# GuoleiSun/VSS-CFFM

Measured on AMD Instinct MI355X. Metric: clips/sec (fwd+bwd) CFFM-B1 480x480 T=4 hot path (CFFA+CFM, decoder_focal depth 2), higher is better.
Workload: dtype f32 in/out, f32 accumulate; MFMA operands: split-bf16 (hi+lo, ~2^-17) in the Linear GEMMs, f16 in QK^T/AV

## Files before the change

### vss_cffm_amd/csrc/cffa_kernels.h

```cpp
#pragma once
#include "cffm_common.h"

__device__ __forceinline__ void transpose_body(const float* __restrict__ src, float* __restrict__ dst,
                                               int rows, int cols, long src_bs, long dst_bs,
                                               const float* __restrict__ addend, int add_mod, int add_skip,
                                               float* __restrict__ copy_dst, int bx, int by, int bz) {
    __shared__ float tile[64][65];
    const int r0 = by * 64, c0 = bx * 64;
    const float* s = src + (long)bz * src_bs;
    float* d = dst + (long)bz * dst_bs;
    const int q = threadIdx.x & 15, p = threadIdx.x >> 4;
    const bool vin = (cols % 4 == 0) && (src_bs % 4 == 0) && (((uintptr_t)src & 15) == 0);
    const bool vout = (rows % 4 == 0) && (dst_bs % 4 == 0) && (((uintptr_t)dst & 15) == 0) && (((uintptr_t)addend & 15) == 0);
    const float* ad = (addend && (bz % add_mod) != add_skip) ? addend + (long)bz * dst_bs : nullptr;
    float* cp = (copy_dst && (bz % add_mod) != add_skip) ? copy_dst + (long)bz * src_bs : nullptr;
#pragma unroll
    for (int k = 0; k < 4; ++k) {
        const int r = r0 + p + 16 * k, c = c0 + 4 * q;
        f32x4 v = (f32x4){0.f, 0.f, 0.f, 0.f};
        if (r < rows) {
            if (vin && c + 3 < cols) {
                v = *(const f32x4*)(s + (long)r * cols + c);
                if (cp) *(f32x4*)(cp + (long)r * cols + c) = v;
            } else
// ... 265 lines not shown
    }
    f32x4 ag = (f32x4){0.f, 0.f, 0.f, 0.f}, ab = (f32x4){0.f, 0.f, 0.f, 0.f};
    __syncthreads();
#pragma unroll
    for (int k = 0; k < LNB_PIX; ++k) {
        const int i = s + LNB_SPLIT * (wave + LNB_WAVES * k);
        if (i >= CFFM_WA) break;
        const int y = 7 * wy + i / 7, x = 7 * wx + i % 7;
        if (!((y < G.H0) && (x < G.W0))) continue;
        const long pix = (long)y * G.W0 + x;
        const float rs = rsr[k];
        const f32x4 xh = (xr[k] - mur[k]) * rs;
        const f32x4 z = xh * gm + bt;
        const f32x4 dz = dzr[k] + m0[k] * dp;
        const float dm = wave_sum_hi(dot4(dp, z));
        if (lane == 63) sdM[i] = dm;
        ag += dz * xh;
        ab += dz;
        const f32x4 gz = dz * gm;
        const float m1 = wave_sum(gz[0] + gz[1] + gz[2] + gz[3]) * (1.f / CFFM_C);
        const float m2 = wave_sum(dot4(gz, xh)) * (1.f / CFFM_C);
        const f32x4 dx = (gz - m1 - xh * m2) * rs + addr[k];
        *(f32x4*)(dxf + pix * CFFM_C + 4 * lane) = dx;
    }
    *(f32x4*)(&red[wave][0][4 * lane]) = ag;
    *(f32x4*)(&red[wave][1][4 * lane]) = ab;
    __syncthreads();
    float* r = rec + (long)blockIdx.x * LNP_RSTRIDE;
    for (int e = threadIdx.x; e < 2 * CFFM_C; e += LNB_THREADS) {
        const int which = e / CFFM_C, ch = e % CFFM_C;
        float t = red[0][which][ch];
#pragma unroll
        for (int q = 1; q < LNB_WAVES; ++q) t += red[q][which][ch];
        r[e] = t;
    }
    if (threadIdx.x < CFFM_WA) r[2 * CFFM_C + threadIdx.x] = sdM[threadIdx.x];
    if (threadIdx.x == CFFM_WA) r[2 * CFFM_C + CFFM_WA] = sbs;
}

#define RB_MAXD 4
struct CffaRefBlocks {
    int n;
    const float* gamma[RB_MAXD];
    const float* beta[RB_MAXD];
    const float* M[RB_MAXD];
    const float* dzall[RB_MAXD];
    float* rec[RB_MAXD];
};
#define RB_LDS_BLOCK (14 * CFFM_C + 2 * 14 * CFFM_WA)
__host__ __device__ constexpr int cffa_ref_lds(int D) {
    return 4 * ((D * RB_LDS_BLOCK > LNB_WAVES * D * 2 * CFFM_C + 14 * D * CFFM_WA ? D * RB_LDS_BLOCK : LNB_WAVES * D * 2 * CFFM_C + 14 * D * CFFM_WA) + 4 * D + 4);
}

struct RefRows { f32x4 x[LNB_PIX], add[LNB_PIX]; float mu[LNB_PIX], rs[LNB_PIX]; };
template <bool ACC>
__device__ __forceinline__ void ln_pool_ref_load(RefRows& R, const Geo& G, const float* __restrict__ xf, const float* __restrict__ dxf,
                                                 const float* __restrict__ mean_f, const float* __restrict__ rstd_f, int s, int wy, int wx,
                                                 int lane, int wave) {
#pragma unroll
    for (int k = 0; k < LNB_PIX; ++k) {
        const int i = s + LNB_SPLIT * (wave + LNB_WAVES * k);
        const int y = 7 * wy + i / 7, x = 7 * wx + i % 7;
        R.x[k] = R.add[k] = (f32x4){0.f, 0.f, 0.f, 0.f};
        R.mu[k] = R.rs[k] = 0.f;
        if (i < CFFM_WA && y < G.H0 && x < G.W0) {
            const long pix = (long)y * G.W0 + x;
            R.x[k] = *(const f32x4*)(xf + pix * CFFM_C + 4 * lane);
            R.mu[k] = mean_f[pix];
            R.rs[k] = rstd_f[pix];
            if (ACC) R.add[k] = *(const f32x4*)(dxf + pix * CFFM_C + 4 * lane);
        }
    }
}
template <int NC, int D>
__device__ __forceinline__ void ln_pool_bwd_ref_frame(const Geo& G, const RefRows& R, float* __restrict__ dxf,
                                                      const float* sP, const float* sMm, float* sdM, const f32x4 (&gm)[D], const f32x4 (&bt)[D],
                                                      f32x4 (&ag)[D], f32x4 (&ab)[D], int g0, int s, int wy, int wx, int lane, int wave) {
#pragma unroll
    for (int k = 0; k < LNB_PIX; ++k) {
        const int i = s + LNB_SPLIT * (wave + LNB_WAVES * k);
        if (i >= CFFM_WA) break;
        const int y = 7 * wy + i / 7, x = 7 * wx + i % 7;
        if (!((y < G.H0) && (x < G.W0))) continue;
        const long pix = (long)y * G.W0 + x;
        const float rs = R.rs[k];
        const f32x4 xh = (R.x[k] - R.mu[k]) * rs;
        f32x4 gz = (f32x4){0.f, 0.f, 0.f, 0.f};
        constexpr int NCD = NC == 9 ? 3 : (NC == 4 ? 2 : 1), WSG = NC == 9 ? 2 : (NC == 4 ? 3 : 7);
        const int iy = i / 7, ix = i % 7;
        int u0 = 0, u1 = 0, v0 = 0, v1 = 0;
        if (NC > 1) {
            u0 = (iy > 0 ? iy - 1 : 0) / WSG; u1 = (iy < 5 ? iy : 5) / WSG;
            v0 = (ix > 0 ? ix - 1 : 0) / WSG; v1 = (ix < 5 ? ix : 5) / WSG;
        }
#pragma unroll
        for (int d = 0; d < D; ++d) {
            const f32x4 z = xh * gm[d] + bt[d];
            f32x4 dz = (f32x4){0.f, 0.f, 0.f, 0.f};
            for (int u = u0; u <= u1; ++u)
                for (int v = v0; v <= v1; ++v) {
                    const int c = d * 14 + g0 - 1 + u * NCD + v;
                    const f32x4 dp = *(const f32x4*)(sP + c * CFFM_C + 4 * lane);
                    dz += sMm[c * CFFM_WA + i] * dp;
                    const float dm = wave_sum_hi(dot4(dp, z));
                    if (lane == 63) sdM[c * CFFM_WA + i] = dm;
                }
            ag[d] += dz * xh;
            ab[d] += dz;
            gz += dz * gm[d];
        }
        const float m1 = wave_sum(gz[0] + gz[1] + gz[2] + gz[3]) * (1.f / CFFM_C);
        const float m2 = wave_sum(dot4(gz, xh)) * (1.f / CFFM_C);
        const f32x4 dx = (gz - m1 - xh * m2) * rs + R.add[k];
        *(f32x4*)(dxf + pix * CFFM_C + 4 * lane) = dx;
    }
}

template <int D, bool ACC>
__global__ void __launch_bounds__(LNB_THREADS) k_ln_pool_bwd_ref(Geo G, const float* __restrict__ x_ref, long ref_bs, CffaRefBlocks Bk,
                                                                 const float* __restrict__ mean_in, const float* __restrict__ rstd_in,
                                                                 float* __restrict__ dx_ref, long dref_bs) {
    CFFM_DYN_SMEM(smem);
    float* sP = (float*)smem;
    float* sMm = sP + D * 14 * CFFM_C;
    float* red = (float*)smem;
    constexpr int body = D * (14 * CFFM_C + 14 * CFFM_WA), redn = LNB_WAVES * D * 2 * CFFM_C;
    float* sdM = (float*)smem + (body > redn ? body : redn);
    float* sbs = sdM + D * 14 * CFFM_WA;
    const int s = blockIdx.x % LNB_SPLIT, wb = blockIdx.x / LNB_SPLIT;
    const int w = wb % G.nW, b = wb / G.nW;
    const int wy = w / G.gx, wx = w % G.gx;
    const int lane = threadIdx.x & 63, wave = wave_uniform(threadIdx.x >> 6);
    for (int e = threadIdx.x; e < D * 14 * CFFM_WA; e += LNB_THREADS) {
        const int d = e / (14 * CFFM_WA), r = e % (14 * CFFM_WA);
        sMm[e] = Bk.M[d][CFFM_WA + r];
        sdM[e] = 0.f;
    }
    for (int r = wave; r < D * 14; r += LNB_WAVES) {
        const int d = r / 14, c = r % 14;
        *(f32x4*)(sP + r * CFFM_C + 4 * lane) = *(const f32x4*)(Bk.dzall[d] + ((long)b * G.RC + cell_row(G, wy, wx, 1 + c)) * CFFM_C + 4 * lane);
    }
    f32x4 gm[D], bt[D], ag[D], ab[D];
#pragma unroll
    for (int d = 0; d < D; ++d) {
        gm[d] = *(const f32x4*)(Bk.gamma[d] + 4 * lane);
        bt[d] = *(const f32x4*)(Bk.beta[d] + 4 * lane);
        ag[d] = ab[d] = (f32x4){0.f, 0.f, 0.f, 0.f};
    }
    __syncthreads();
    if (s == 0) {
        for (int q = wave; q < 3 * D; q += LNB_WAVES) {
            const int d = q / 3, grp = q % 3;
            const int c0 = grp == 0 ? 0 : (grp == 1 ? 1 : 5), nc = grp == 0 ? 1 : (grp == 1 ? 4 : 9);
            float t = 0.f;
            for (int c = 0; c < nc; ++c) {
                const f32x4 v = *(const f32x4*)(sP + (d * 14 + c0 + c) * CFFM_C + 4 * lane);
                t += v[0] + v[1] + v[2] + v[3];
            }
            t = wave_sum(t);
            if (lane == 0) sbs[d * 4 + grp] = t;
        }
    } else if (threadIdx.x < 4 * D) sbs[threadIdx.x] = 0.f;
    const float* xb = x_ref + (long)b * ref_bs;
    float* dxb = dx_ref + (long)b * dref_bs;
    const long fr = (long)G.HW * CFFM_C;
    const float* mb = mean_in + (long)b * 4 * G.HW;
    const float* rb = rstd_in + (long)b * 4 * G.HW;
    RefRows Ra, Rb;
    ln_pool_ref_load<ACC>(Ra, G, xb, dxb, mb, rb, s, wy, wx, lane, wave);
    ln_pool_ref_load<ACC>(Rb, G, xb + fr, dxb + fr, mb + G.HW, rb + G.HW, s, wy, wx, lane, wave);
    ln_pool_bwd_ref_frame<1, D>(G, Ra, dxb, sP, sMm, sdM, gm, bt, ag, ab, 1, s, wy, wx, lane, wave);
    ln_pool_ref_load<ACC>(Ra, G, xb + 2 * fr, dxb + 2 * fr, mb + 2 * G.HW, rb + 2 * G.HW, s, wy, wx, lane, wave);
    ln_pool_bwd_ref_frame<4, D>(G, Rb, dxb + fr, sP, sMm, sdM, gm, bt, ag, ab, 2, s, wy, wx, lane, wave);
    ln_pool_bwd_ref_frame<9, D>(G, Ra, dxb + 2 * fr, sP, sMm, sdM, gm, bt, ag, ab, 6, s, wy, wx, lane, wave);
    __syncthreads();
#pragma unroll
    for (int d = 0; d < D; ++d) {
        *(f32x4*)(red + ((wave * D + d) * 2 + 0) * CFFM_C + 4 * lane) = ag[d];
        *(f32x4*)(red + ((wave * D + d) * 2 + 1) * CFFM_C + 4 * lane) = ab[d];
    }
    __syncthreads();
    for (int d = 0; d < D; ++d) {
        float* r = Bk.rec[d] + (long)blockIdx.x * LNP_RSTRIDE;
        for (int e = threadIdx.x; e < 2 * CFFM_C; e += LNB_THREADS) {
            float t = red[(d * 2) * CFFM_C + e];
#pragma unroll
            for (int q = 1; q < LNB_WAVES; ++q) t += red[((q * D + d) * 2) * CFFM_C + e];
            r[e] = t;
        }
        for (int e = threadIdx.x; e < LNP_TAIL_REF; e += LNB_THREADS)
            r[2 * CFFM_C + e] = e < 14 * CFFM_WA ? sdM[d * 14 * CFFM_WA + e] : sbs[d * 4 + (e - 14 * CFFM_WA)];
    }
}
```

### vss_cffm_amd/csrc/cffm_hip.hip

```cpp
#include "cfm_attn_kernels.h"
#include "clip_kernels.h"
#include "rowops_kernels.h"
#include "gtc_kernels.h"
#include "gemm.h"
#include "segfuse_kernels.h"
#include "segloss_kernels.h"
#include "headfuse_kernels.h"
#include "kmeans_kernels.h"
#include "predict_kernels.h"
#include "mixffn_kernels.h"
#include "sra_kernels.h"
#include "srln_kernels.h"
#include "mitln_kernels.h"

#include <stdarg.h>
#include <stdio.h>

#include "../../include/cffm_hip.h"

static thread_local char g_err[512] = "";

static int fail(int code, const char* fmt, ...) {
    va_list ap;
    va_start(ap, fmt);
// ... 589 lines not shown
}
int cffm_add_inplace(float* a, const float* b, long n, void* stream) {
    REQUIRE(a && b && n >= 0 && n % 4 == 0, "add_inplace: n must be a multiple of 4");
    if (!n) return 0;
    CFFM_LAUNCH(k_add_inplace, (ew_grid(n / 4)), (256), 0, (hipStream_t)stream, a, b, n / 4);
    CHECK_LAUNCH("add_inplace");
    return 0;
}
int cffm_transpose(const float* src, float* dst, int batch, int rows, int cols, long src_bs, long dst_bs, void* stream) {
    return transpose_add(src, dst, batch, rows, cols, src_bs, dst_bs, nullptr, 1, -1, stream);
}

int cffm_pool_matrix(const float* const pool_w[4], float* M, void* stream) {
    PROF(ST_POOLMAT);
    PoolW pw;
    for (int i = 0; i < 4; ++i) { REQUIRE(pool_w[i], "pool_matrix: null weight %d", i); pw.w[i] = pool_w[i]; }
    CFFM_LAUNCH(k_pool_matrix, (1), (256), 0, (hipStream_t)stream, pw, M);
    CHECK_LAUNCH("pool_matrix");
    return 0;
}

static thread_local int g_grad_pads = 0;
void cffm_grad_slices_padded(int yes) { g_grad_pads = yes ? 1 : 0; }

static int ln_pool_fwd_impl(const cffm_geom* g, const float* x_ref, long ref_bs, const float* x_tgt, long tgt_bs,
                            const float* gamma, const float* beta, const float* M, const float* const pool_b[4],
                            float* zall, float* mean, float* rstd, int split, void* stream, const float* const* pool_w = nullptr) {
    PROF(ST_LN_POOL_FWD);
    REQUIRE(g && x_ref && x_tgt && zall, "ln_pool_fwd: null");
    PoolB pb;
    PoolW pw;
    for (int i = 0; i < 4; ++i) { pb.b[i] = pool_b[i]; pw.w[i] = pool_w ? pool_w[i] : nullptr; }
    CFFM_LAUNCH(k_ln_pool_fwd<false>, (g->nW, 4, g->B), (LNP_THREADS), 0, (hipStream_t)stream, to_geo(g), x_ref, ref_bs, x_tgt, tgt_bs, gamma,
                beta, pool_w ? nullptr : M, pw, pb, zall, mean, rstd, split);
    CHECK_LAUNCH("ln_pool_fwd");
    return 0;
}
int cffm_ln_pool_fwd(const cffm_geom* g, const float* x_ref, long ref_bs, const float* x_tgt, long tgt_bs,
                     const float* gamma, const float* beta, const float* M, const float* const pool_b[4],
                     float* zall, float* mean, float* rstd, void* stream) {
    return ln_pool_fwd_impl(g, x_ref, ref_bs, x_tgt, tgt_bs, gamma, beta, M, pool_b, zall, mean, rstd, 0, stream);
}

static long cffa_rows(const cffm_geom* g) { return (long)g->B * g->nW * LNB_SPLIT; }
static int ln_pool_bwd_tgt(const cffm_geom* g, const float* x_tgt, long tgt_bs, const float* gamma, const float* beta, const float* M,
                           const float* mean, const float* rstd, const float* dzall, const float* dres, float* dx_tgt, long dtgt_bs,
                           float* rec, void* stream) {
    PROF(ST_LN_POOL_BWD);
    CFFM_LAUNCH(k_ln_pool_bwd_tgt, ((unsigned)cffa_rows(g)), (LNB_THREADS), 0, (hipStream_t)stream, to_geo(g), x_tgt, tgt_bs, gamma, beta, M, mean, rstd,
                dzall, dres, dx_tgt, dtgt_bs, rec);
    CHECK_LAUNCH("ln_pool_bwd_tgt");
    return 0;
}
extern "C++" {
template <int D>
static int ln_pool_bwd_ref_d(const cffm_geom* g, const float* x_ref, long ref_bs, const CffaRefBlocks& Bk, const float* mean, const float* rstd,
                             float* dx_ref, long dref_bs, int accum, hipStream_t st) {
    constexpr int lds = cffa_ref_lds(D);
#ifndef CFFM_EMU
    static bool granted = false;
    if (!granted && lds > 64 * 1024) {
        if (hipFuncSetAttribute((const void*)k_ln_pool_bwd_ref<D, false>, hipFuncAttributeMaxDynamicSharedMemorySize, lds) != hipSuccess ||
            hipFuncSetAttribute((const void*)k_ln_pool_bwd_ref<D, true>, hipFuncAttributeMaxDynamicSharedMemorySize, lds) != hipSuccess) return -1;
        granted = true;
    }
#endif
    if (accum) CFFM_LAUNCH((k_ln_pool_bwd_ref<D, true>), ((unsigned)cffa_rows(g)), (LNB_THREADS), lds, st, to_geo(g), x_ref, ref_bs, Bk, mean, rstd, dx_ref, dref_bs);
    else CFFM_LAUNCH((k_ln_pool_bwd_ref<D, false>), ((unsigned)cffa_rows(g)), (LNB_THREADS), lds, st, to_geo(g), x_ref, ref_bs, Bk, mean, rstd, dx_ref, dref_bs);
    return 0;
}
}
static int ln_pool_bwd_ref(const cffm_geom* g, const float* x_ref, long ref_bs, const CffaRefBlocks& Bk, const float* mean, const float* rstd,
                           float* dx_ref, long dref_bs, int accum, void* stream) {
    PROF(ST_LN_POOL_BWD_REF);
    hipStream_t st = (hipStream_t)stream;
    int rc = -1;
    switch (Bk.n) {
        case 1: rc = ln_pool_bwd_ref_d<1>(g, x_ref, ref_bs, Bk, mean, rstd, dx_ref, dref_bs, accum, st); break;
        case 2: rc = ln_pool_bwd_ref_d<2>(g, x_ref, ref_bs, Bk, mean, rstd, dx_ref, dref_bs, accum, st); break;
        case 3: rc = ln_pool_bwd_ref_d<3>(g, x_ref, ref_bs, Bk, mean, rstd, dx_ref, dref_bs, accum, st); break;
        case 4: rc = ln_pool_bwd_ref_d<4>(g, x_ref, ref_bs, Bk, mean, rstd, dx_ref, dref_bs, accum, st); break;
        default: break;
    }
    REQUIRE(!rc, "ln_pool_bwd_ref: bad block count %d or LDS grant failed", Bk.n);
    CHECK_LAUNCH("ln_pool_bwd_ref");
    return 0;
}
static void job_add(RedJobs& J, const float* part, int nblk, int stride, int total, const RedSegs& segs, hipStream_t st) {
    if (J.njob == RED_MAXJOB) redq_launch(J, st);
    const int j = J.njob++;
    J.part[j] = part; J.nblk[j] = nblk; J.stride[j] = stride; J.total[j] = total; J.segs[j] = segs;
    J.blk_end[j] = (j ? J.blk_end[j - 1] : 0) + (total + 63) / 64;
}
static void cffa_jobs(RedJobs& J, const float* rec, long rows, float* dgamma, float* dbeta, float* dM, float* const dpool_b[4], hipStream_t st) {
    RedSegs a, b, c;
    a.nseg = b.nseg = c.nseg = 0;
    seg_add(a, 0, CFFM_C, dgamma, 0);
    seg_add(a, CFFM_C, CFFM_C, dbeta, 0);
    job_add(J, rec, (int)(2 * rows), LNP_RSTRIDE, 2 * CFFM_C, a, st);
    seg_add(b, 0, CFFM_WA, dM, 0);
    seg_add(b, CFFM_WA, 1, dpool_b[0], 0);
    job_add(J, rec + 2 * CFFM_C, (int)rows, LNP_RSTRIDE, LNP_TAIL_TGT, b, st);
    seg_add(c, 0, 14 * CFFM_WA, dM + CFFM_WA, 0);
    for (int i = 1; i < 4; ++i) seg_add(c, 14 * CFFM_WA + i - 1, 1, dpool_b[i], 0);
    job_add(J, rec + rows * LNP_RSTRIDE + 2 * CFFM_C, (int)rows, LNP_RSTRIDE, LNP_TAIL_REF, c, st);
}

static float* g_scr4 = nullptr;
static size_t g_scr4_floats = 0;
static float* lib_scratch4(size_t nfloats) {
    if (nfloats <= g_scr4_floats) return g_scr4;
#ifdef CFFM_EMU
    free(g_scr4);
    g_scr4 = (float*)malloc(nfloats * sizeof(float));
#else
    if (g_scr4) { (void)hipDeviceSynchronize(); (void)hipFree(g_scr4); }
    if (hipMalloc((void**)&g_scr4, nfloats * sizeof(float)) != hipSuccess) g_scr4 = nullptr;
#endif
    g_scr4_floats = g_scr4 ? nfloats : 0;
    return g_scr4;
}
struct CffaSlot { float* dzall; float* rec; float* dM; };
static int cffa_slot(const cffm_geom* g, int slot, int nslots, CffaSlot* o) {
    const long a = up((long)g->B * g->RC * CFFM_C), b = up(2 * cffa_rows(g) * LNP_RSTRIDE), c = up(CFFM_NCELL * CFFM_WA);
    float* base = lib_scratch4((size_t)(a + b + c) * nslots);
    REQUIRE(base && slot >= 0 && slot < nslots, "cffa: scratch allocation failed");
    float* p = base + (a + b + c) * slot;
    o->dzall = p; o->rec = p + a; o->dM = p + a + b;
    return 0;
}
static int cffa_finish(const cffm_geom* g, int nslots, const cffm_block_params* params, const cffm_block_grads* grads, int first, int last,
                       const float* ws0, long ws_stride, const float* x_ref, long ref_bs, float* dx_ref, long dref_bs, int accum, void* stream,
                       RedJobs* extra = nullptr) {
    cffm_block_ws L;
    cffm_block_ws_layout(g, &L);
    hipStream_t st = (hipStream_t)stream;
    const long rows = cffa_rows(g);
    static_assert(PMB_MAXD == RB_MAXD, "one pooling-matrix launch per reference launch");
    for (int hi = first; hi >= last; hi -= RB_MAXD) {
        const int n = hi - last + 1 < RB_MAXD ? hi - last + 1 : RB_MAXD;
        CffaRefBlocks Bk;
        PoolWGN pw;
        RedJobs J;
        Bk.n = n; J.njob = 0;
        for (int d = 0; d < RB_MAXD; ++d) {
            const int i = hi - (d < n ? d : 0);
            CffaSlot S;
            TRY(cffa_slot(g, i, nslots, &S));
            Bk.gamma[d] = params[i].norm1_w; Bk.beta[d] = params[i].norm1_b; Bk.M[d] = ws0 + i * ws_stride + L.M;
            Bk.dzall[d] = S.dzall; Bk.rec[d] = S.rec + rows * LNP_RSTRIDE;
            pw.dM[d] = S.dM;
            for (int q = 0; q < 4; ++q) { pw.gw[d].w[q] = grads[i].pool_w[q]; pw.gw[d].b[q] = g_grad_pads ? grads[i].pool_b[q] : nullptr; }
        }
        const float* ws = ws0 + (long)hi * ws_stride;
        TRY(ln_pool_bwd_ref(g, x_ref, ref_bs, Bk, ws + L.mean1, ws + L.rstd1, dx_ref, dref_bs, accum || hi != first, stream));
        for (int d = 0; d < n; ++d) {
            const int i = hi - d;
            CffaSlot S;
            TRY(cffa_slot(g, i, nslots, &S));
            cffa_jobs(J, S.rec, rows, grads[i].norm1_w, grads[i].norm1_b, S.dM, grads[i].pool_b, st);
        }
        if (extra && hi - RB_MAXD < last) {
            for (int j = 0; j < extra->njob; ++j) job_add(J, extra->part[j], extra->nblk[j], extra->stride[j], extra->total[j], extra->segs[j], st);
            extra->njob = 0;
        }
        redq_launch(J, st);
        CHECK_LAUNCH("cffa reductions");
        {
            PROF(ST_POOLMAT);
            CFFM_LAUNCH(k_pool_matrix_bwd_n, (111, n), (64), 0, st, pw);
            CHECK_LAUNCH("pool_matrix_bwd");
        }
    }
    return 0;
}

int cffm_bias_assemble(const float* own, const float* ring, const float* const pool[4], float* bias, void* biasH, void* stream) {
    PROF(ST_BIAS_ASM);
    BiasTables t;
    t.own = own; t.ring = ring;
    for (int i = 0; i < 4; ++i) t.pool[i] = pool[i];
    const int n = CFFM_HEADS * CFFM_NQ_PAD * CFFM_NKEY_PAD;
    CFFM_LAUNCH(k_bias_assemble, ((n + 255) / 256), (256), 0, (hipStream_t)stream, t, bias, (h16*)biasH);
    CHECK_LAUNCH("bias_assemble");
    return 0;
}

static int cffm_bias_scatter(const float* dbiasT, float* down, float* dring, float* const dpool[4], void* stream) {
    PROF(ST_BIAS_SCT);
    BiasTablesG t;
    t.own = down; t.ring = dring;
    for (int i = 0; i < 4; ++i) t.pool[i] = dpool[i];
    CFFM_LAUNCH(k_bias_scatter, ((BIAS_SCATTER_THREADS + 255) / 256), (256), 0, (hipStream_t)stream, dbiasT, t);
    CHECK_LAUNCH("bias_scatter");
    return 0;
}

int cffm_attn_fwd(const cffm_geom* g, const void* qkv16, const int* key_src, const int* q_dst, const void* biasH, float* ao,
                  float* lse, void* stream) {
    PROF(ST_ATTN_FWD);
    REQUIRE(g && qkv16 && key_src && q_dst && biasH && ao && lse, "attn_fwd: null");
    const h16* bias = (const h16*)biasH;
    CFFM_LAUNCH(k_cfm_attn_fwd<false>, (g->B * g->nW * CFFM_HEADS), (256), ATT_FWD_LDS, (hipStream_t)stream, to_geo(g), (const h16*)qkv16,
                key_src, q_dst, bias, ao, lse);
    CHECK_LAUNCH("attn_fwd");
    return 0;
}

static int attn_bwd_groups(const cffm_geom* g, int* per_group) {
    const int total = g->B * g->nW;
    const int ng = total < 32 ? total : 32;
    *per_group = (total + ng - 1) / ng;
    return (total + *per_group - 1) / *per_group;
// ... 597 lines not shown
    TRY(cffm_attn_fwd(g, ws + L.qkv, key_src, q_dst, (const void*)(ws + L.bias), ws + L.ao, ws + L.lse, stream));
    {
        const float* wf = ws + L.w_frag;
        PROF(ST_GEMM);
        if (dw_stream_sw())
            TRY(cffm_mlp_fwd_tfrag(ws + L.ao, x_tgt, tgt_bs, g->HW, wf + 768 * 256, wf + 768 * 256 + 256 * 256, wf + 768 * 256 + 256 * 256 + 1024 * 256,
                                   p->proj_b, p->fc1_b, p->fc2_b, p->norm2_w, p->norm2_b, ws + L.x1, nullptr, ws + L.mean2, ws + L.rstd2, ws + L.hraw,
                                   nullptr, ws + L.x2, ws + L.ao_t, ws + L.z2, ws + L.act, NP, stream));
        else
        TRY(cffm_mlp_fwd(ws + L.ao, x_tgt, tgt_bs, g->HW, wf + 768 * 256, wf + 768 * 256 + 256 * 256, wf + 768 * 256 + 256 * 256 + 1024 * 256,
                         p->proj_b, p->fc1_b, p->fc2_b, p->norm2_w, p->norm2_b, ws + L.x1, ws + L.z2, ws + L.mean2, ws + L.rstd2, ws + L.hraw,
                         ws + L.act, ws + L.x2, NP, stream));
        CHECK_LAUNCH("block_forward");
    }
    (void)scratch;
    return 0;
}

static int block_backward_impl(const cffm_geom* g, const cffm_block_params* p, const cffm_block_grads* gr,
                               const float* x_ref, long ref_bs, const float* x_tgt, long tgt_bs, const int* key_src,
                               const int* q_dst, const int* inv_ptr, const int* inv_idx, const float* ws, const float* dout,
                               float* dx_tgt, long dtgt_bs, float* scratch, int defer, int par, int slot, int nslots, void* stream);
#ifndef CFFM_EMU
static struct { bool has; RedJobs jobs; int parity; } g_tail = {false, {}, 0};
static int tail_flush(hipStream_t st) {
    if (!g_tail.has) return 0;
    g_tail.has = false;
    hipStream_t s3 = side_fork_take(st, 3);
    (void)hipStreamWaitEvent(s3, g_side.tail_order, 0);
    redq_launch(g_tail.jobs, s3);
    CHECK_LAUNCH("block_backward reductions");
    if (s3 != st) {
        side_record(s3, st, g_side.tail_done[g_tail.parity]);
        g_side.tail_pending[g_tail.parity] = true;
    }
    return 0;
}
#else
static int tail_flush(hipStream_t) { return 0; }
#endif
static void tail_reset() {
#ifndef CFFM_EMU
    g_tail.has = false;
    for (int i = 0; i < 2; ++i) g_side.dw_pending[i] = g_side.bias_pending[i] = g_side.tail_pending[i] = false;
#endif
}
int cffm_block_backward(const cffm_geom* g, const cffm_block_params* p, const cffm_block_grads* gr,
                        const float* x_ref, long ref_bs, const float* x_tgt, long tgt_bs, const int* key_src,
                        const int* q_dst, const int* inv_ptr, const int* inv_idx, const float* ws, const float* dout,
                        float* dx_ref, long dref_bs, int accum_ref, float* dx_tgt, long dtgt_bs, float* scratch, void* stream) {
    REQUIRE(x_ref && dx_ref, "block_backward: null");
    TRY(block_backward_impl(g, p, gr, x_ref, ref_bs, x_tgt, tgt_bs, key_src, q_dst, inv_ptr, inv_idx, ws, dout, dx_tgt, dtgt_bs, scratch, 0, 0, 0, 1,
                            stream));
    return cffa_finish(g, 1, p, gr, 0, 0, ws, 0, x_ref, ref_bs, dx_ref, dref_bs, accum_ref, stream);
}
static int block_backward_impl(const cffm_geom* g, const cffm_block_params* p, const cffm_block_grads* gr,
                               const float* x_ref, long ref_bs, const float* x_tgt, long tgt_bs, const int* key_src,
                               const int* q_dst, const int* inv_ptr, const int* inv_idx, const float* ws, const float* dout,
                               float* dx_tgt, long dtgt_bs, float* scratch, int defer, int par, int slot, int nslots, void* stream) {
    REQUIRE(g && p && gr && ws && dout && scratch, "block_backward: null");
    cffm_block_ws L;
    cffm_block_ws_layout(g, &L);
    const Scratch S = scratch_layout(g);
    const long NR = (long)g->B * g->RC, NP = (long)g->B * g->HW;
    par = (defer && par) ? 1 : 0;
    const long altb = S.alt, altact = altb + up(NP * CFFM_C), altqkv = altact + up((NP + 31) / 32 * 32 * CFFM_HID), altbias = altqkv + up(NR * 768);
    float* dx1 = scratch + (par ? altb : S.b);
    float* dz2 = scratch + S.dz2;
    float* dao = scratch + S.dao;
    float* dact = scratch + (par ? altact : S.dact);
    float* dqkv = scratch + (par ? altqkv : S.dqkv);
    const long NP32 = (NP + 31) / 32 * 32;
    float* dout_t = scratch + S.tf + (par ? S.tf_stride : 0);
    float* dx1_t = dout_t + up(NP32 * CFFM_C);
    float* dqkv_t = dx1_t + up(NP32 * CFFM_C);
    const int stream_dw = dw_stream_sw();
    CffaSlot cffa;
    TRY(cffa_slot(g, slot, nslots, &cffa));
    float* dzall = cffa.dzall;
    float* dbiasT = scratch + (par ? altbias : S.dbiasT);
    RedScope reductions((hipStream_t)stream);
    hipStream_t st = (hipStream_t)stream;
    hipStream_t sa = st;
    side_init(st);
#ifndef CFFM_EMU
    if (g_side.tail_pending[g_red_parity]) {
        side_wait(st, g_side.tail_done[g_red_parity]);
        g_side.tail_pending[g_red_parity] = false;
    }
    g_side.par = par;
    if (g_side.dw_pending[par]) {
        side_wait(st, g_side.dw_done[par]);
        g_side.dw_pending[par] = false;
    }
#endif
    const int one_group = dw_one_group(st);
    if (!one_group) {
        const GemmTN all4[4] = {{nullptr, nullptr, nullptr, NR, 768, CFFM_C}, {nullptr, nullptr, nullptr, NP, CFFM_HID, CFFM_C},
                                {nullptr, nullptr, nullptr, NP, CFFM_C, CFFM_HID}, {nullptr, nullptr, nullptr, NP, CFFM_C, CFFM_C}};
        size_t need = gemm_tn_group_partial_floats(all4, 4, 480);
        DwsPlan P4;
        if (stream_dw && dw_stream_plan(all4, 4, dw_stream_target(), &P4)) need = P4.part_floats;
        REQUIRE(!need || lib_scratch2(need), "block_backward: scratch allocation failed");
    }
    auto dw_group = [&](const cffm_wgrad* wg, const GemmTNPre* pre, int n, hipStream_t s, int target, void (*after)(hipStream_t)) -> int {
        if (!stream_dw) return gemm_tn_group((const GemmTN*)wg, n, s, pre, s == st ? lib_scratch : lib_scratch2, target, after);
        DwsPlan P;
// ... 552 lines not shown
    CHECK_LAUNCH("vc_counts");
    return 0;
}

int cffm_layer_forward_rows(const cffm_geom* g, int depth, const cffm_block_params* params, const float* x_rows, float* y_rows,
                            const int* key_src, const int* q_dst, float* saved, float* scratch, void* stream) {
    REQUIRE(g && params && x_rows && y_rows && saved && scratch && depth >= 1, "layer_forward_rows: bad arguments");
    cffm_block_ws L;
    cffm_block_ws_layout(g, &L);
    const long HW = g->HW, img = HW * CFFM_C;
    float* blk0 = saved + up((long)g->B * 4 * img);
    TRY(param_prep(params, depth, blk0, L.total, L, stream));
    for (int i = 0; i < depth; ++i) {
        float* ws = blk0 + (long)i * L.total;
        const float* tgt = (i == 0) ? x_rows + 3 * img : blk0 + (long)(i - 1) * L.total + L.x2;
        const long tgt_bs = (i == 0) ? 4 * img : img;
        TRY(block_forward_impl(g, &params[i], x_rows, 4 * img, tgt, tgt_bs, key_src, q_dst, ws, scratch, stream));
    }
#ifdef CFFM_EMU
    memcpy(y_rows, blk0 + (long)(depth - 1) * L.total + L.x2, (size_t)g->B * img * sizeof(float));
#else
    REQUIRE(hipMemcpyAsync(y_rows, blk0 + (long)(depth - 1) * L.total + L.x2, (size_t)g->B * img * sizeof(float), hipMemcpyDeviceToDevice,
                           (hipStream_t)stream) == hipSuccess, "layer_forward_rows: copy failed");
#endif
    return 0;
}
int cffm_layer_backward_rows(const cffm_geom* g, int depth, const cffm_block_params* params, const cffm_block_grads* grads,
                             const float* x_rows, const float* dy_rows, float* dx_rows, const int* key_src, const int* q_dst,
                             const int* inv_ptr, const int* inv_idx, const float* saved, float* scratch, void* stream) {
    REQUIRE(g && params && grads && x_rows && dy_rows && dx_rows && saved && scratch && depth >= 1, "layer_backward_rows: bad arguments");
    cffm_block_ws L;
    cffm_block_ws_layout(g, &L);
    const Scratch S = scratch_layout(g);
    const long HW = g->HW, img = HW * CFFM_C;
    const float* blk0 = saved + up((long)g->B * 4 * img);
    tail_reset();
    for (int i = depth - 1; i >= 0; --i) {
        const float* ws = blk0 + (long)i * L.total;
        const float* tgt = (i == 0) ? x_rows + 3 * img : blk0 + (long)(i - 1) * L.total + L.x2;
        const long tgt_bs = (i == 0) ? 4 * img : img;
        float* dtgt = (i == 0) ? dx_rows + 3 * img : scratch + (((depth - i) & 1) ? S.a2 : S.a);
        const long dtgt_bs = (i == 0) ? 4 * img : img;
        const float* dout = (i == depth - 1) ? dy_rows : scratch + (((depth - 1 - i) & 1) ? S.a2 : S.a);
        TRY(block_backward_impl(g, &params[i], &grads[i], x_rows, 4 * img, tgt, tgt_bs, key_src, q_dst, inv_ptr, inv_idx, ws, dout, dtgt, dtgt_bs,
                                scratch, 1, (depth - 1 - i) & 1, i, depth, stream));
    }
    RedJobs* tail_jobs = nullptr;
#ifndef CFFM_EMU
    if (g_tail.has) {
        g_tail.has = false;
        tail_jobs = &g_tail.jobs;
    }
#endif
    TRY(cffa_finish(g, depth, params, grads, depth - 1, 0, blk0, L.total, x_rows, 4 * img, dx_rows, 4 * img, 0, stream, tail_jobs));
    side_join_all((hipStream_t)stream);
    return 0;
}

static int layer_forward_impl(const cffm_geom* g, int depth, const cffm_block_params* params, const float* x_nchw,
                              float* y_tgt_nchw, long y_bs, float* y_full, const int* key_src, const int* q_dst, float* saved,
                              float* scratch, void* stream) {
    REQUIRE(g && params && x_nchw && y_tgt_nchw && saved && scratch && depth >= 1, "layer_forward: bad arguments");
    cffm_block_ws L;
    cffm_block_ws_layout(g, &L);
    const long HW = g->HW, img = HW * CFFM_C;
    float* xs = saved;
    float* blk0 = saved + up((long)g->B * 4 * img);
    hipStream_t st = (hipStream_t)stream;
    side_init(st);
    if (depth <= PREP_MAXD) {
        PROF(ST_TRANSPOSE);
        PrepArgs a;
        const int pnx = prep_args(a, params, 0, depth, blk0, L.total, L);
        TrArgs T;
        T.src = x_nchw; T.dst = xs; T.rows = CFFM_C; T.cols = (int)HW; T.src_bs = img; T.dst_bs = img; T.add_mod = 4; T.add_skip = 3; T.copy_dst = y_full;
        T.gx = ((int)HW + 63) / 64; T.gy = (CFFM_C + 63) / 64; T.gz = g->B * 4;
        CFFM_LAUNCH(k_transpose_prep, ((unsigned)(T.gx * T.gy * T.gz + pnx * depth)), (256), 0, st, T, a, pnx);
        CHECK_LAUNCH("transpose + param_prep");
        g_prep_join.pending = false;
    } else {
        side_fork_mark(st, 0);
        TRY(transpose_add(x_nchw, xs, g->B * 4, CFFM_C, (int)HW, img, img, nullptr, 4, 3, stream, y_full));
        hipStream_t sd = side_fork_take(st, 0);
        TRY(param_prep(params, depth, blk0, L.total, L, (void*)sd));
        side_mark(sd, st, 0);
        g_prep_join.pending = sd != st;
        g_prep_join.side = sd;
    }
#ifndef CFFM_EMU
    g_side.used = 0;
#endif
    for (int i = 0; i < depth; ++i) {
        float* ws = blk0 + (long)i * L.total;
        const float* tgt = (i == 0) ? xs + 3 * img : blk0 + (long)(i - 1) * L.total + L.x2;
        const long tgt_bs = (i == 0) ? 4 * img : img;
        TRY(block_forward_impl(g, &params[i], xs, 4 * img, tgt, tgt_bs, key_src, q_dst, ws, scratch, stream));
    }
    TRY(cffm_transpose(blk0 + (long)(depth - 1) * L.total + L.x2, y_tgt_nchw, g->B, (int)HW, CFFM_C, img, y_bs, stream));
    return 0;
}
int cffm_layer_forward(const cffm_geom* g, int depth, const cffm_block_params* params, const float* x_nchw,
                       float* y_tgt_nchw, const int* key_src, const int* q_dst, float* saved, float* scratch,
                       void* stream) {
    REQUIRE(g, "layer_forward: bad arguments");
    return layer_forward_impl(g, depth, params, x_nchw, y_tgt_nchw, g->HW * CFFM_C, nullptr, key_src, q_dst, saved, scratch, stream);
}
int cffm_layer_forward_full(const cffm_geom* g, int depth, const cffm_block_params* params, const float* x_nchw,
// ... 133 lines not shown
    TRY(layer_infer_check(g, depth, params, prepared, x_rows, y_rows, key_src, q_dst, ws, "layer_infer_rows"));
    return layer_infer_blocks(g, depth, params, prepared, x_rows, y_rows, key_src, q_dst, ws, stream);
}
int cffm_layer_infer_full(const cffm_geom* g, int depth, const cffm_block_params* params, const float* prepared, const float* x_nchw,
                          float* y_full_nchw, const int* key_src, const int* q_dst, float* ws, void* stream) {
    TRY(layer_infer_check(g, depth, params, prepared, x_nchw, y_full_nchw, key_src, q_dst, ws, "layer_infer_full"));
    const InferWs W = infer_ws_layout(g);
    const long HW = g->HW, img = HW * CFFM_C;
    float* stack = y_full_nchw;
    TRY(transpose_add(x_nchw, stack, g->B * 4, CFFM_C, (int)HW, img, img, nullptr, 1, -1, stream));
    float* last = ws + W.x2[(depth - 1) & 1];
    TRY(layer_infer_blocks(g, depth, params, prepared, stack, last, key_src, q_dst, ws, stream));
    for (int b = 0; b < g->B; ++b)
        REQUIRE(hipMemcpyAsync(y_full_nchw + (long)b * 4 * img, x_nchw + (long)b * 4 * img, (size_t)3 * img * sizeof(float), hipMemcpyDeviceToDevice,
                               (hipStream_t)stream) == hipSuccess, "layer_infer_full: copy failed");
    TRY(cffm_transpose(last, y_full_nchw + 3 * img, g->B, (int)HW, CFFM_C, img, 4 * img, stream));
    return 0;
}

static int layer_backward_impl(const cffm_geom* g, int depth, const cffm_block_params* params, const cffm_block_grads* grads,
                               const float* dy_tgt_nchw, long dy_bs, const float* dy_full, float* dx_nchw, const int* key_src,
                               const int* q_dst, const int* inv_ptr, const int* inv_idx, const float* saved, float* scratch,
                               int first_block, int last_block, void* stream) {
    REQUIRE(g && params && grads && dy_tgt_nchw && dx_nchw && saved && scratch && depth >= 1, "layer_backward: bad arguments");
    REQUIRE(first_block < depth && last_block >= 0 && first_block >= last_block, "layer_backward: bad block range %d..%d of %d", first_block,
            last_block, depth);
    cffm_block_ws L;
    cffm_block_ws_layout(g, &L);
    const Scratch S = scratch_layout(g);
    const long HW = g->HW, img = HW * CFFM_C;
    const float* xs = saved;
    const float* blk0 = saved + up((long)g->B * 4 * img);
    float* dxs = scratch + S.dxs;
    REQUIRE(dy_bs >= img, "layer_backward: dy batch stride %ld < %ld", dy_bs, img);
    if (first_block == depth - 1) TRY(cffm_transpose(dy_tgt_nchw, scratch + S.a, g->B, CFFM_C, (int)HW, dy_bs, img, stream));
    tail_reset();
    for (int i = first_block; i >= last_block; --i) {
        const float* ws = blk0 + (long)i * L.total;
        const float* tgt = (i == 0) ? xs + 3 * img : blk0 + (long)(i - 1) * L.total + L.x2;
        const long tgt_bs = (i == 0) ? 4 * img : img;
        float* dcur = scratch + (((depth - 1 - i) & 1) ? S.a2 : S.a);
        float* dtgt = (i == 0) ? dxs + 3 * img : scratch + (((depth - i) & 1) ? S.a2 : S.a);
        const long dtgt_bs = (i == 0) ? 4 * img : img;
        TRY(block_backward_impl(g, &params[i], &grads[i], xs, 4 * img, tgt, tgt_bs, key_src, q_dst, inv_ptr, inv_idx, ws, dcur, dtgt, dtgt_bs, scratch,
                                1, (depth - 1 - i) & 1, i, depth, stream));
    }
    RedJobs* tail_jobs = nullptr;
#ifndef CFFM_EMU
    if (last_block == 0 && g_tail.has) {
        g_tail.has = false;
        tail_jobs = &g_tail.jobs;
    }
#endif
    TRY(cffa_finish(g, depth, params, grads, first_block, last_block, blk0, L.total, xs, 4 * img, dxs, 4 * img, first_block != depth - 1, stream, tail_jobs));
    if (last_block == 0) TRY(transpose_add(dxs, dx_nchw, g->B * 4, (int)HW, CFFM_C, img, img, dy_full, 4, 3, stream));
    TRY(tail_flush((hipStream_t)stream));
    side_join_all((hipStream_t)stream);
    return 0;
}
int cffm_layer_backward_range(const cffm_geom* g, int depth, const cffm_block_params* params, const cffm_block_grads* grads,
                              const float* dy_tgt_nchw, long dy_bs, float* dx_nchw, const int* key_src, const int* q_dst,
                              const int* inv_ptr, const int* inv_idx, const float* saved, float* scratch, int first_block,
                              int last_block, void* stream) {
    return layer_backward_impl(g, depth, params, grads, dy_tgt_nchw, dy_bs, nullptr, dx_nchw, key_src, q_dst, inv_ptr, inv_idx, saved,
                               scratch, first_block, last_block, stream);
}
int cffm_layer_backward_full(const cffm_geom* g, int depth, const cffm_block_params* params, const cffm_block_grads* grads,
                             const float* dy_full_nchw, float* dx_nchw, const int* key_src, const int* q_dst, const int* inv_ptr,
                             const int* inv_idx, const float* saved, float* scratch, int first_block, int last_block, void* stream) {
    REQUIRE(g && dy_full_nchw && dy_full_nchw != dx_nchw, "layer_backward_full: bad arguments");
    const long img = g->HW * CFFM_C;
    return layer_backward_impl(g, depth, params, grads, dy_full_nchw + 3 * img, 4 * img, dy_full_nchw, dx_nchw, key_src, q_dst, inv_ptr,
                               inv_idx, saved, scratch, first_block, last_block, stream);
}
int cffm_layer_backward(const cffm_geom* g, int depth, const cffm_block_params* params, const cffm_block_grads* grads,
                        const float* dy_tgt_nchw, long dy_bs, float* dx_nchw, const int* key_src, const int* q_dst,
                        const int* inv_ptr, const int* inv_idx, const float* saved, float* scratch, void* stream) {
    return cffm_layer_backward_range(g, depth, params, grads, dy_tgt_nchw, dy_bs, dx_nchw, key_src, q_dst, inv_ptr, inv_idx, saved, scratch,
                                     depth - 1, 0, stream);
}

}
struct KmPlan { int KT, tpw, P; size_t frag_b, part_b, cnt_b; };
static KmPlan km_plan(long N, int K) {
    KmPlan p;
    p.KT = (K + 15) / 16;
    const long tiles = (N + 15) / 16;
    long tpw = (tiles + 4L * KM_WGS - 1) / (4L * KM_WGS);
    if (tpw < 1) tpw = 1;
    if (tpw > KM_MAX_TPW) tpw = KM_MAX_TPW;
    p.tpw = (int)tpw;
    p.P = (int)((N + 64 * tpw - 1) / (64 * tpw));
    p.frag_b = (size_t)km_frag_words(p.KT) * 16;
    p.part_b = ((size_t)p.P * K * CFFM_C * 4 + 255) / 256 * 256;
    p.cnt_b = ((size_t)p.P * K * 4 + 255) / 256 * 256;
    return p;
}
static int km_check(const char* who, long N, int K) {
    REQUIRE(K >= 1 && K <= 128, "%s: K=%d outside 1..128", who, K);
    REQUIRE(N >= K && N <= (1L << 30), "%s: N=%ld outside K..2^30 (K=%d)", who, N, K);
    return 0;
}
template <int KT>
static int km_run(const float* x, int N, int K, int iters, float* centers, int* labels, int* counts, char* ws, const KmPlan& p, hipStream_t st) {
    const size_t lds = (size_t)km_step_lds(KT, p.tpw);
#ifndef CFFM_EMU
    static size_t granted = 0;
// ... 453 lines not shown
```

Measured before the change: 2884.

## Choose ref LN-pool backward split per launch from an occupancy model

Makes the per-window split factor of the reference-frame LN/pool backward kernel a template parameter (3 or 4). A host-side cost model built from hard-coded VGPR counts, LDS use, CU count and whether it runs beside a depthwise kernel picks the split with the fewest waves times pixels per thread. Mean and rstd are packed into one f32x2 per pixel, and the reduction job row counts now follow the chosen split. This trades more grid parallelism against per-thread serial work, relies on register numbers measured offline, and adds an env override and more template instances.

After: 2879. No clear change (-0.2%).

```diff
diff --git a/vss_cffm_amd/csrc/cffa_kernels.h b/vss_cffm_amd/csrc/cffa_kernels.h
--- a/vss_cffm_amd/csrc/cffa_kernels.h
+++ b/vss_cffm_amd/csrc/cffa_kernels.h
@@ -341,39 +341,40 @@
     return 4 * ((D * RB_LDS_BLOCK > LNB_WAVES * D * 2 * CFFM_C + 14 * D * CFFM_WA ? D * RB_LDS_BLOCK : LNB_WAVES * D * 2 * CFFM_C + 14 * D * CFFM_WA) + 4 * D + 4);
 }
 
-struct RefRows { f32x4 x[LNB_PIX], add[LNB_PIX]; float mu[LNB_PIX], rs[LNB_PIX]; };
-template <bool ACC>
-__device__ __forceinline__ void ln_pool_ref_load(RefRows& R, const Geo& G, const float* __restrict__ xf, const float* __restrict__ dxf,
+__host__ __device__ constexpr int lnb_ref_pix(int split) { return (CFFM_WA + split * LNB_WAVES - 1) / (split * LNB_WAVES); }
+template <int SPLIT>
+struct RefRows { f32x4 x[lnb_ref_pix(SPLIT)], add[lnb_ref_pix(SPLIT)]; f32x2 ms[lnb_ref_pix(SPLIT)]; };
+template <bool ACC, int SPLIT>
+__device__ __forceinline__ void ln_pool_ref_load(RefRows<SPLIT>& R, const Geo& G, const float* __restrict__ xf, const float* __restrict__ dxf,
                                                  const float* __restrict__ mean_f, const float* __restrict__ rstd_f, int s, int wy, int wx,
                                                  int lane, int wave) {
 #pragma unroll
-    for (int k = 0; k < LNB_PIX; ++k) {
-        const int i = s + LNB_SPLIT * (wave + LNB_WAVES * k);
+    for (int k = 0; k < lnb_ref_pix(SPLIT); ++k) {
+        const int i = s + SPLIT * (wave + LNB_WAVES * k);
         const int y = 7 * wy + i / 7, x = 7 * wx + i % 7;
         R.x[k] = R.add[k] = (f32x4){0.f, 0.f, 0.f, 0.f};
-        R.mu[k] = R.rs[k] = 0.f;
+        R.ms[k] = (f32x2){0.f, 0.f};
         if (i < CFFM_WA && y < G.H0 && x < G.W0) {
             const long pix = (long)y * G.W0 + x;
             R.x[k] = *(const f32x4*)(xf + pix * CFFM_C + 4 * lane);
-            R.mu[k] = mean_f[pix];
-            R.rs[k] = rstd_f[pix];
+            R.ms[k] = (f32x2){mean_f[pix], rstd_f[pix]};
             if (ACC) R.add[k] = *(const f32x4*)(dxf + pix * CFFM_C + 4 * lane);
         }
     }
 }
-template <int NC, int D>
-__device__ __forceinline__ void ln_pool_bwd_ref_frame(const Geo& G, const RefRows& R, float* __restrict__ dxf,
+template <int NC, int D, int SPLIT>
+__device__ __forceinline__ void ln_pool_bwd_ref_frame(const Geo& G, const RefRows<SPLIT>& R, float* __restrict__ dxf,
                                                       const float* sP, const float* sMm, float* sdM, const f32x4 (&gm)[D], const f32x4 (&bt)[D],
                                                       f32x4 (&ag)[D], f32x4 (&ab)[D], int g0, int s, int wy, int wx, int lane, int wave) {
 #pragma unroll
-    for (int k = 0; k < LNB_PIX; ++k) {
-        const int i = s + LNB_SPLIT * (wave + LNB_WAVES * k);
+    for (int k = 0; k < lnb_ref_pix(SPLIT); ++k) {
+        const int i = s + SPLIT * (wave + LNB_WAVES * k);
         if (i >= CFFM_WA) break;
         const int y = 7 * wy + i / 7, x = 7 * wx + i % 7;
         if (!((y < G.H0) && (x < G.W0))) continue;
         const long pix = (long)y * G.W0 + x;
-        const float rs = R.rs[k];
-        const f32x4 xh = (R.x[k] - R.mu[k]) * rs;
+        const float mu = R.ms[k][0], rs = R.ms[k][1];
+        const f32x4 xh = (R.x[k] - mu) * rs;
         f32x4 gz = (f32x4){0.f, 0.f, 0.f, 0.f};
         constexpr int NCD = NC == 9 ? 3 : (NC == 4 ? 2 : 1), WSG = NC == 9 ? 2 : (NC == 4 ? 3 : 7);
         const int iy = i / 7, ix = i % 7;
@@ -405,7 +406,7 @@
     }
 }
 
-template <int D, bool ACC>
+template <int D, bool ACC, int SPLIT>
 __global__ void __launch_bounds__(LNB_THREADS) k_ln_pool_bwd_ref(Geo G, const float* __restrict__ x_ref, long ref_bs, CffaRefBlocks Bk,
                                                                  const float* __restrict__ mean_in, const float* __restrict__ rstd_in,
                                                                  float* __restrict__ dx_ref, long dref_bs) {
@@ -416,7 +417,7 @@
     constexpr int body = D * (14 * CFFM_C + 14 * CFFM_WA), redn = LNB_WAVES * D * 2 * CFFM_C;
     float* sdM = (float*)smem + (body > redn ? body : redn);
     float* sbs = sdM + D * 14 * CFFM_WA;
-    const int s = blockIdx.x % LNB_SPLIT, wb = blockIdx.x / LNB_SPLIT;
+    const int s = blockIdx.x % SPLIT, wb = blockIdx.x / SPLIT;
     const int w = wb % G.nW, b = wb / G.nW;
     const int wy = w / G.gx, wx = w % G.gx;
     const int lane = threadIdx.x & 63, wave = wave_uniform(threadIdx.x >> 6);
@@ -455,13 +456,13 @@
     const long fr = (long)G.HW * CFFM_C;
     const float* mb = mean_in + (long)b * 4 * G.HW;
     const float* rb = rstd_in + (long)b * 4 * G.HW;
-    RefRows Ra, Rb;
-    ln_pool_ref_load<ACC>(Ra, G, xb, dxb, mb, rb, s, wy, wx, lane, wave);
-    ln_pool_ref_load<ACC>(Rb, G, xb + fr, dxb + fr, mb + G.HW, rb + G.HW, s, wy, wx, lane, wave);
-    ln_pool_bwd_ref_frame<1, D>(G, Ra, dxb, sP, sMm, sdM, gm, bt, ag, ab, 1, s, wy, wx, lane, wave);
-    ln_pool_ref_load<ACC>(Ra, G, xb + 2 * fr, dxb + 2 * fr, mb + 2 * G.HW, rb + 2 * G.HW, s, wy, wx, lane, wave);
-    ln_pool_bwd_ref_frame<4, D>(G, Rb, dxb + fr, sP, sMm, sdM, gm, bt, ag, ab, 2, s, wy, wx, lane, wave);
-    ln_pool_bwd_ref_frame<9, D>(G, Ra, dxb + 2 * fr, sP, sMm, sdM, gm, bt, ag, ab, 6, s, wy, wx, lane, wave);
+    RefRows<SPLIT> Ra, Rb;
+    ln_pool_ref_load<ACC, SPLIT>(Ra, G, xb, dxb, mb, rb, s, wy, wx, lane, wave);
+    ln_pool_ref_load<ACC, SPLIT>(Rb, G, xb + fr, dxb + fr, mb + G.HW, rb + G.HW, s, wy, wx, lane, wave);
+    ln_pool_bwd_ref_frame<1, D, SPLIT>(G, Ra, dxb, sP, sMm, sdM, gm, bt, ag, ab, 1, s, wy, wx, lane, wave);
+    ln_pool_ref_load<ACC, SPLIT>(Ra, G, xb + 2 * fr, dxb + 2 * fr, mb + 2 * G.HW, rb + 2 * G.HW, s, wy, wx, lane, wave);
+    ln_pool_bwd_ref_frame<4, D, SPLIT>(G, Rb, dxb + fr, sP, sMm, sdM, gm, bt, ag, ab, 2, s, wy, wx, lane, wave);
+    ln_pool_bwd_ref_frame<9, D, SPLIT>(G, Ra, dxb + 2 * fr, sP, sMm, sdM, gm, bt, ag, ab, 6, s, wy, wx, lane, wave);
     __syncthreads();
 #pragma unroll
     for (int d = 0; d < D; ++d) {
diff --git a/vss_cffm_amd/csrc/cffm_hip.hip b/vss_cffm_amd/csrc/cffm_hip.hip
--- a/vss_cffm_amd/csrc/cffm_hip.hip
+++ b/vss_cffm_amd/csrc/cffm_hip.hip
@@ -665,37 +665,95 @@
     CHECK_LAUNCH("ln_pool_bwd_tgt");
     return 0;
 }
+#define REF_DW_VGPR 256
+#define REF_DW_LDS 75776
+#define REF_CU_VGPR 512
+#define REF_CU_LDS 163840
+static const int REF_VGPR[2][RB_MAXD][2] = {
+    {{82, 122}, {104, 0}, {123, 0}, {0, 0}},
+    {{74, 106}, {95, 127}, {114, 148}, {134, 166}},
+};
+static constexpr bool cffa_ref_split3(int D, bool accum) { return D == 1 || (D < RB_MAXD && !accum); }
+static bool cffa_ref_eligible(int split, int D, int accum) { return split == 4 || (split == 3 && cffa_ref_split3(D, accum != 0)); }
+static int cffa_ref_slots(int split, int D, int accum, int beside_dw) {
+    const int vg = (REF_VGPR[split == 3 ? 0 : 1][D - 1][accum ? 1 : 0] + 7) / 8 * 8;
+    const int by_regs = ((beside_dw ? REF_CU_VGPR - REF_DW_VGPR : REF_CU_VGPR) / vg) * 4 / LNB_WAVES;
+    const int by_lds = (beside_dw ? REF_CU_LDS - REF_DW_LDS : REF_CU_LDS) / cffa_ref_lds(D);
+    const int n = by_regs < by_lds ? by_regs : by_lds;
+    return n < 1 ? 1 : n;
+}
+static int device_cus() {
+#ifdef CFFM_EMU
+    return 256;
+#else
+    static int cus = 0;
+    if (!cus) {
+        int dev = 0;
+        hipDeviceProp_t pr;
+        cus = (hipGetDevice(&dev) == hipSuccess && hipGetDeviceProperties(&pr, dev) == hipSuccess && pr.multiProcessorCount > 0) ? pr.multiProcessorCount : 256;
+        (void)hipGetLastError();
+    }
+    return cus;
+#endif
+}
+static int cffa_ref_split(const cffm_geom* g, int D, int accum, int beside_dw) {
+    const char* e = getenv("CFFM_REF_SPLIT");
+    if (e && (e[0] == '3' || e[0] == '4') && !e[1] && cffa_ref_eligible(e[0] - '0', D, accum)) return e[0] - '0';
+    long best = 0;
+    int pick = LNB_SPLIT;
+    for (int split = LNB_SPLIT; split >= 3; --split) {
+        if (!cffa_ref_eligible(split, D, accum)) continue;
+        const long wgs = (long)g->B * g->nW * split, places = (long)cffa_ref_slots(split, D, accum, beside_dw) * device_cus();
+        const long cost = ((wgs + places - 1) / places) * lnb_ref_pix(split);
+        if (!best || cost < best) { best = cost; pick = split; }
+    }
+    return pick;
+}
 extern "C++" {
+template <int D, int SPLIT>
+static int ln_pool_bwd_ref_ds(const cffm_geom* g, const float* x_ref, long ref_bs, const CffaRefBlocks& Bk, const float* mean, const float* rstd,
+                              float* dx_ref, long dref_bs, int accum, hipStream_t st) {
+    constexpr int lds = cffa_ref_lds(D);
+#ifndef CFFM_EMU
+    static bool granted = false;
+    if constexpr (lds > 64 * 1024) {
+        if (!granted) {
+            if (hipFuncSetAttribute((const void*)k_ln_pool_bwd_ref<D, false, SPLIT>, hipFuncAttributeMaxDynamicSharedMemorySize, lds) != hipSuccess ||
+                hipFuncSetAttribute((const void*)k_ln_pool_bwd_ref<D, true, SPLIT>, hipFuncAttributeMaxDynamicSharedMemorySize, lds) != hipSuccess) return -1;
+            granted = true;
+        }
+    }
+#endif
+    const unsigned grid = (unsigned)((long)g->B * g->nW * SPLIT);
+    if (accum) {
+        if constexpr (SPLIT == 4 || cffa_ref_split3(D, true))
+            CFFM_LAUNCH((k_ln_pool_bwd_ref<D, true, SPLIT>), (grid), (LNB_THREADS), lds, st, to_geo(g), x_ref, ref_bs, Bk, mean, rstd, dx_ref, dref_bs);
+        else return -1;
+    } else CFFM_LAUNCH((k_ln_pool_bwd_ref<D, false, SPLIT>), (grid), (LNB_THREADS), lds, st, to_geo(g), x_ref, ref_bs, Bk, mean, rstd, dx_ref, dref_bs);
+    return 0;
+}
 template <int D>
 static int ln_pool_bwd_ref_d(const cffm_geom* g, const float* x_ref, long ref_bs, const CffaRefBlocks& Bk, const float* mean, const float* rstd,
-                             float* dx_ref, long dref_bs, int accum, hipStream_t st) {
-    constexpr int lds = cffa_ref_lds(D);
-#ifndef CFFM_EMU
-    static bool granted = false;
-    if (!granted && lds > 64 * 1024) {
-        if (hipFuncSetAttribute((const void*)k_ln_pool_bwd_ref<D, false>, hipFuncAttributeMaxDynamicSharedMemorySize, lds) != hipSuccess ||
-            hipFuncSetAttribute((const void*)k_ln_pool_bwd_ref<D, true>, hipFuncAttributeMaxDynamicSharedMemorySize, lds) != hipSuccess) return -1;
-        granted = true;
-    }
-#endif
-    if (accum) CFFM_LAUNCH((k_ln_pool_bwd_ref<D, true>), ((unsigned)cffa_rows(g)), (LNB_THREADS), lds, st, to_geo(g), x_ref, ref_bs, Bk, mean, rstd, dx_ref, dref_bs);
-    else CFFM_LAUNCH((k_ln_pool_bwd_ref<D, false>), ((unsigned)cffa_rows(g)), (LNB_THREADS), lds, st, to_geo(g), x_ref, ref_bs, Bk, mean, rstd, dx_ref, dref_bs);
-    return 0;
+                             float* dx_ref, long dref_bs, int accum, int split, hipStream_t st) {
+    if constexpr (cffa_ref_split3(D, false))
+        if (split == 3) return ln_pool_bwd_ref_ds<D, 3>(g, x_ref, ref_bs, Bk, mean, rstd, dx_ref, dref_bs, accum, st);
+    if (split == 4) return ln_pool_bwd_ref_ds<D, 4>(g, x_ref, ref_bs, Bk, mean, rstd, dx_ref, dref_bs, accum, st);
+    return -1;
 }
 }
 static int ln_pool_bwd_ref(const cffm_geom* g, const float* x_ref, long ref_bs, const CffaRefBlocks& Bk, const float* mean, const float* rstd,
-                           float* dx_ref, long dref_bs, int accum, void* stream) {
+                           float* dx_ref, long dref_bs, int accum, int split, void* stream) {
     PROF(ST_LN_POOL_BWD_REF);
     hipStream_t st = (hipStream_t)stream;
     int rc = -1;
     switch (Bk.n) {
-        case 1: rc = ln_pool_bwd_ref_d<1>(g, x_ref, ref_bs, Bk, mean, rstd, dx_ref, dref_bs, accum, st); break;
-        case 2: rc = ln_pool_bwd_ref_d<2>(g, x_ref, ref_bs, Bk, mean, rstd, dx_ref, dref_bs, accum, st); break;
-        case 3: rc = ln_pool_bwd_ref_d<3>(g, x_ref, ref_bs, Bk, mean, rstd, dx_ref, dref_bs, accum, st); break;
-        case 4: rc = ln_pool_bwd_ref_d<4>(g, x_ref, ref_bs, Bk, mean, rstd, dx_ref, dref_bs, accum, st); break;
+        case 1: rc = ln_pool_bwd_ref_d<1>(g, x_ref, ref_bs, Bk, mean, rstd, dx_ref, dref_bs, accum, split, st); break;
+        case 2: rc = ln_pool_bwd_ref_d<2>(g, x_ref, ref_bs, Bk, mean, rstd, dx_ref, dref_bs, accum, split, st); break;
+        case 3: rc = ln_pool_bwd_ref_d<3>(g, x_ref, ref_bs, Bk, mean, rstd, dx_ref, dref_bs, accum, split, st); break;
+        case 4: rc = ln_pool_bwd_ref_d<4>(g, x_ref, ref_bs, Bk, mean, rstd, dx_ref, dref_bs, accum, split, st); break;
         default: break;
     }
-    REQUIRE(!rc, "ln_pool_bwd_ref: bad block count %d or LDS grant failed", Bk.n);
+    REQUIRE(!rc, "ln_pool_bwd_ref: bad block count %d, split %d, or LDS grant failed", Bk.n, split);
     CHECK_LAUNCH("ln_pool_bwd_ref");
     return 0;
 }
@@ -705,18 +763,18 @@
     J.part[j] = part; J.nblk[j] = nblk; J.stride[j] = stride; J.total[j] = total; J.segs[j] = segs;
     J.blk_end[j] = (j ? J.blk_end[j - 1] : 0) + (total + 63) / 64;
 }
-static void cffa_jobs(RedJobs& J, const float* rec, long rows, float* dgamma, float* dbeta, float* dM, float* const dpool_b[4], hipStream_t st) {
+static void cffa_jobs(RedJobs& J, const float* rec, long rows, long rows_ref, float* dgamma, float* dbeta, float* dM, float* const dpool_b[4], hipStream_t st) {
     RedSegs a, b, c;
     a.nseg = b.nseg = c.nseg = 0;
     seg_add(a, 0, CFFM_C, dgamma, 0);
     seg_add(a, CFFM_C, CFFM_C, dbeta, 0);
-    job_add(J, rec, (int)(2 * rows), LNP_RSTRIDE, 2 * CFFM_C, a, st);
+    job_add(J, rec, (int)(rows + rows_ref), LNP_RSTRIDE, 2 * CFFM_C, a, st);
     seg_add(b, 0, CFFM_WA, dM, 0);
     seg_add(b, CFFM_WA, 1, dpool_b[0], 0);
     job_add(J, rec + 2 * CFFM_C, (int)rows, LNP_RSTRIDE, LNP_TAIL_TGT, b, st);
     seg_add(c, 0, 14 * CFFM_WA, dM + CFFM_WA, 0);
     for (int i = 1; i < 4; ++i) seg_add(c, 14 * CFFM_WA + i - 1, 1, dpool_b[i], 0);
-    job_add(J, rec + rows * LNP_RSTRIDE + 2 * CFFM_C, (int)rows, LNP_RSTRIDE, LNP_TAIL_REF, c, st);
+    job_add(J, rec + rows * LNP_RSTRIDE + 2 * CFFM_C, (int)rows_ref, LNP_RSTRIDE, LNP_TAIL_REF, c, st);
 }
 
 static float* g_scr4 = nullptr;
@@ -744,7 +802,7 @@
 }
 static int cffa_finish(const cffm_geom* g, int nslots, const cffm_block_params* params, const cffm_block_grads* grads, int first, int last,
                        const float* ws0, long ws_stride, const float* x_ref, long ref_bs, float* dx_ref, long dref_bs, int accum, void* stream,
-                       RedJobs* extra = nullptr) {
+                       int beside_dw, RedJobs* extra = nullptr) {
     cffm_block_ws L;
     cffm_block_ws_layout(g, &L);
     hipStream_t st = (hipStream_t)stream;
@@ -756,6 +814,8 @@
         PoolWGN pw;
         RedJobs J;
         Bk.n = n; J.njob = 0;
+        const int acc = accum || hi != first, split = cffa_ref_split(g, n, acc, beside_dw);
+        const long rows_ref = (long)g->B * g->nW * split;
         for (int d = 0; d < RB_MAXD; ++d) {
             const int i = hi - (d < n ? d : 0);
             CffaSlot S;
@@ -766,12 +826,12 @@
             for (int q = 0; q < 4; ++q) { pw.gw[d].w[q] = grads[i].pool_w[q]; pw.gw[d].b[q] = g_grad_pads ? grads[i].pool_b[q] : nullptr; }
         }
         const float* ws = ws0 + (long)hi * ws_stride;
-        TRY(ln_pool_bwd_ref(g, x_ref, ref_bs, Bk, ws + L.mean1, ws + L.rstd1, dx_ref, dref_bs, accum || hi != first, stream));
+        TRY(ln_pool_bwd_ref(g, x_ref, ref_bs, Bk, ws + L.mean1, ws + L.rstd1, dx_ref, dref_bs, acc, split, stream));
         for (int d = 0; d < n; ++d) {
             const int i = hi - d;
             CffaSlot S;
             TRY(cffa_slot(g, i, nslots, &S));
-            cffa_jobs(J, S.rec, rows, grads[i].norm1_w, grads[i].norm1_b, S.dM, grads[i].pool_b, st);
+            cffa_jobs(J, S.rec, rows, rows_ref, grads[i].norm1_w, grads[i].norm1_b, S.dM, grads[i].pool_b, st);
         }
         if (extra && hi - RB_MAXD < last) {
             for (int j = 0; j < extra->njob; ++j) job_add(J, extra->part[j], extra->nblk[j], extra->stride[j], extra->total[j], extra->segs[j], st);
@@ -1475,7 +1535,7 @@
     REQUIRE(x_ref && dx_ref, "block_backward: null");
     TRY(block_backward_impl(g, p, gr, x_ref, ref_bs, x_tgt, tgt_bs, key_src, q_dst, inv_ptr, inv_idx, ws, dout, dx_tgt, dtgt_bs, scratch, 0, 0, 0, 1,
                             stream));
-    return cffa_finish(g, 1, p, gr, 0, 0, ws, 0, x_ref, ref_bs, dx_ref, dref_bs, accum_ref, stream);
+    return cffa_finish(g, 1, p, gr, 0, 0, ws, 0, x_ref, ref_bs, dx_ref, dref_bs, accum_ref, stream, 0);
 }
 static int block_backward_impl(const cffm_geom* g, const cffm_block_params* p, const cffm_block_grads* gr,
                                const float* x_ref, long ref_bs, const float* x_tgt, long tgt_bs, const int* key_src,
@@ -2134,7 +2194,7 @@
         tail_jobs = &g_tail.jobs;
     }
 #endif
-    TRY(cffa_finish(g, depth, params, grads, depth - 1, 0, blk0, L.total, x_rows, 4 * img, dx_rows, 4 * img, 0, stream, tail_jobs));
+    TRY(cffa_finish(g, depth, params, grads, depth - 1, 0, blk0, L.total, x_rows, 4 * img, dx_rows, 4 * img, 0, stream, 1, tail_jobs));
     side_join_all((hipStream_t)stream);
     return 0;
 }
@@ -2374,7 +2434,7 @@
         tail_jobs = &g_tail.jobs;
     }
 #endif
-    TRY(cffa_finish(g, depth, params, grads, first_block, last_block, blk0, L.total, xs, 4 * img, dxs, 4 * img, first_block != depth - 1, stream, tail_jobs));
+    TRY(cffa_finish(g, depth, params, grads, first_block, last_block, blk0, L.total, xs, 4 * img, dxs, 4 * img, first_block != depth - 1, stream, 1, tail_jobs));
     if (last_block == 0) TRY(transpose_add(dxs, dx_nchw, g->B * 4, (int)HW, CFFM_C, img, img, dy_full, 4, 3, stream));
     TRY(tail_flush((hipStream_t)stream));
     side_join_all((hipStream_t)stream);
```
